# AkshayThiru/distributed-aerial-transportation

Measured on AMD Instinct MI355X. Metric: agent-QP solves/sec (node) + ms per control step, 6-quad C-ADMM, 1/2/4/8 GPU, higher is better.
Workload: dtype f64

## Files before the change

distributed_aerial_transportation_amd/_lib.py:

```python

from __future__ import annotations

import ctypes
import hashlib
import os
import subprocess

import numpy as np

PKG = os.path.dirname(os.path.abspath(__file__))
REPO = os.path.dirname(PKG)
LIB_PATH = os.path.join(PKG, "libdat.so")
SRC = os.path.join(PKG, "csrc", "dat.hip")
SRC_CENT = os.path.join(PKG, "csrc", "dat_cent.hip")
SRC_COMM = os.path.join(PKG, "csrc", "dat_comm.hip")
SRCS = (SRC, SRC_CENT, SRC_COMM)
OBJ_DIR = os.path.join(PKG, "build")
HIPFLAGS = ["--offload-arch=gfx950", "-O3", "-std=c++17", "-fPIC", "-ffp-contract=on"]
DEPS = [SRC, SRC_CENT, SRC_COMM, os.path.join(PKG, "csrc", "dat_core.hpp"), os.path.join(PKG, "csrc", "dat_qp.hpp"),
        os.path.join(PKG, "csrc", "dat_cadmm_step.hpp"), os.path.join(PKG, "csrc", "dat_dd_step.hpp"),
        os.path.join(PKG, "csrc", "dat_pmrl_step.hpp"), os.path.join(PKG, "csrc", "dat_kargs.hpp"),
        os.path.join(PKG, "csrc", "dat_ckpt.hpp"),
        os.path.join(PKG, "csrc", "dat_layout.h"), os.path.join(REPO, "include", "dat.h")]

# ... 103 lines not shown
    "dat_create": (ctypes.c_int, [ctypes.POINTER(Config), ctypes.POINTER(H)]),
    "dat_destroy": (ctypes.c_int, [H]),
    "dat_last_error": (ctypes.c_char_p, []),
    "dat_device_count": (ctypes.c_int, []),
    "dat_set_params": (ctypes.c_int, [H, D, ctypes.c_int]),
    "dat_set_forests": (ctypes.c_int, [H, ctypes.c_int, I, D, I, D]),
    "dat_set_tolerance": (ctypes.c_int, [H, ctypes.c_double, ctypes.c_int]),
    "dat_set_max_iter": (ctypes.c_int, [H, ctypes.c_int]),
    "dat_set_qp_tolerance": (ctypes.c_int, [H, ctypes.c_double]),
    "dat_reset_warm_start": (ctypes.c_int, [H]),
    "dat_set_state": (ctypes.c_int, [H, D, I]),
    "dat_get_state": (ctypes.c_int, [H, D, I]),
    "dat_checkpoint_bytes": (ctypes.c_int, [H, ctypes.c_int, LL]),
    "dat_checkpoint_save": (ctypes.c_int, [H, I, ctypes.c_int, ctypes.c_void_p, ctypes.c_longlong]),
    "dat_checkpoint_load": (ctypes.c_int, [H, ctypes.c_void_p, ctypes.c_longlong, I, I, ctypes.c_int]),
    "dat_get_checkpoint_ms": (ctypes.c_int, [H, D, D]),
    "dat_control_step": (ctypes.c_int, [H, D, D, D, I, I, D, U8, D]),
    "dat_rollout": (ctypes.c_int, [H, ctypes.c_int, D]),
    "dat_closed_loop": (ctypes.c_int, [H, ctypes.c_int]),
    "dat_control_steps": (ctypes.c_int, [H, ctypes.c_int, D, D, I, I]),
    "dat_set_sub_batches": (ctypes.c_int, [H, ctypes.c_int]),
    "dat_set_advance_overlap": (ctypes.c_int, [H, ctypes.c_int]),
    "dat_set_step_pipeline": (ctypes.c_int, [H, ctypes.c_int]),
    "dat_get_stream_count": (ctypes.c_int, [H]),
    "dat_get_advance_counts": (ctypes.c_int, [H, LL, LL]),
    "dat_debug_advance_split": (ctypes.c_int, [H, U8]),
    "dat_debug_get_env_class": (ctypes.c_int, [H, D, D, I, I]),
    "dat_get_step_marks": (ctypes.c_int, [H, D, ctypes.c_int]),
    "dat_get_counters": (ctypes.c_int, [H, LL, LL, LL, LL, D]),
    "dat_get_class_counters": (ctypes.c_int, [H, ctypes.c_int, LL, LL, LL, D]),
    "dat_get_class_occupancy": (ctypes.c_int, [H, ctypes.c_int, LL, LL]),
    "dat_reset_counters": (ctypes.c_int, [H]),
    "dat_synchronize": (ctypes.c_int, [H]),
    "dat_set_persistent_blocks": (ctypes.c_int, [H, ctypes.c_int]),
    "dat_cadmm_slots": (ctypes.c_int, [H, ctypes.c_int, I]),
    "dat_cadmm_row_mode": (ctypes.c_int, [ctypes.c_int, ctypes.c_int, ctypes.c_int]),
    "dat_env_rows": (ctypes.c_int, [H, D, D, I, U8, D]),
    "dat_solve_agent_qp_batch": (ctypes.c_int, [H, ctypes.c_int, I, I, D, D, D, D, D, D, I, I, U8, D]),
    "dat_solve_agent_qp_rows_batch": (ctypes.c_int, [H, ctypes.c_int, I, I, D, D, D, D, D, D, D, I, D, I, I, U8, D,
                                                     U8]),
    "dat_set_low_level": (ctypes.c_int, [H, ctypes.c_int]),
    "dat_get_kernel_ms": (ctypes.c_int, [H, D]),
    "dat_get_inband_exits": (ctypes.c_int, [H, LL, LL]),
    "dat_get_refinement_counters": (ctypes.c_int, [H, LL, LL]),
    "dat_get_robust_redos": (ctypes.c_int, [H, LL]),
    "dat_get_tail_counters": (ctypes.c_int, [H, LL]),
# ... 59 lines not shown
```

distributed_aerial_transportation_amd/control.py:

```python

from __future__ import annotations

import ctypes
from dataclasses import dataclass, field
from typing import Any, List, Optional, Tuple

import numpy as np

from . import _lib as L
from . import layout
from .system import (RQPCollision, RQPParameters, RQPState, _skew, equilibrium_forces, pack_mountain, pack_params,
                     pack_state)

MODES = {"centralized": L.MODE_CENTRALIZED, "consensus-admm": L.MODE_CADMM, "cadmm": L.MODE_CADMM,
         "dual-decomposition": L.MODE_DD, "dd": L.MODE_DD}


@dataclass
class SolverStatistics:

    iter: int
    solve_time: float
    collision: bool
    min_env_dist: float
# ... 271 lines not shown
        if f.ndim == 3:
            f = f[None]
        assert f.ndim == 4 and f.shape[1:] == (self.batch, 3, self.n), f.shape
        fd = L.f64(f.transpose(0, 1, 3, 2).reshape(f.shape[0], self.batch, 3 * self.n))
        L.check(self._lib.dat_pmrl_rollout(self._h, int(steps), L.ptr(fd), int(f.shape[0])))

    def pmrl_forward(self, f: np.ndarray):
        B, n = self.batch, self.n
        f = np.asarray(f, float)
        assert f.shape == (B, 3, n), f.shape
        fd = L.f64(f.transpose(0, 2, 1).reshape(B, 3 * n))
        ddq, dvl, dwl, T = np.empty((B, n, 3)), np.empty((B, 3)), np.empty((B, 3)), np.empty((B, n))
        L.check(self._lib.dat_pmrl_forward(self._h, L.ptr(fd), L.ptr(ddq), L.ptr(dvl), L.ptr(dwl), L.ptr(T)))
        return (ddq.transpose(0, 2, 1).copy(), dvl, dwl), T

    def set_sub_batches(self, count: int) -> None:
        L.check(self._lib.dat_set_sub_batches(self._h, int(count)))

    def set_advance_overlap(self, on: bool) -> None:
        L.check(self._lib.dat_set_advance_overlap(self._h, int(bool(on))))

    def set_step_pipeline(self, on: bool) -> None:
        L.check(self._lib.dat_set_step_pipeline(self._h, int(bool(on))))

    def stream_count(self) -> int:
        m = self._lib.dat_get_stream_count(self._h)
        if m < 0:
            L.check(m)
        return m

    def advance_counts(self) -> Tuple[int, int]:
        e, l = ctypes.c_longlong(), ctypes.c_longlong()
        L.check(self._lib.dat_get_advance_counts(self._h, ctypes.byref(e), ctypes.byref(l)))
        return e.value, l.value

    def debug_advance_split(self, early_mask) -> None:
        if early_mask is None:
            L.check(self._lib.dat_debug_advance_split(self._h, None))
            return
        m = np.ascontiguousarray(np.asarray(early_mask) != 0, dtype=np.uint8)
        if m.shape != (self.batch,):
            raise ValueError("early_mask must have one entry per scenario")
        L.check(self._lib.dat_debug_advance_split(self._h, L.ptr(m, L.U8)))

    def debug_env_class(self):
        B, n = self.batch, self.n
# ... 426 lines not shown
```

distributed_aerial_transportation_amd/csrc/dat.hip:

```cpp
#include <hip/hip_runtime.h>

#include <climits>
#include <cmath>
#include <cstdio>
#include <cstring>
#include <cstdlib>
#include <mutex>
#include <string>
#include <type_traits>
#include <vector>
#include <algorithm>
#include <chrono>

#include "../../include/dat.h"
#include "dat_ckpt.hpp"
#include "dat_kargs.hpp"
#include "dat_dd_step.hpp"
#include "dat_pmrl_step.hpp"

using namespace dat;

#ifdef DAT_CAPTURE_LOOSE
namespace dat {
constexpr int CAP_MAX = 64, CAP_DOUBLES = 320;
// ... 156 lines not shown
#pragma unroll
    for (int k = 0; k < ENV_CE; ++k) mine[k] = e[k];
    __syncthreads();
    if (!dead) {
      for (int j = 0; j < n; ++j) {
        const double* q = grp + (size_t)j * ENV_CS;
        if (q[0] == 0.0) continue;
        if (!env_in_cone(cam, q[1], q[2])) continue;
        const double dd = q[3];
        if (dd < ENV_TOUCH) out.collision = 1;
        env_see(seen, dd, q + 4, lhs, rhs);
      }
    }
    __syncthreads();
  }
  if (!dead && seen.cnt > 0 && fr.speed > 0.0) {
    out.min_env_dist = seen.dmin;
    *mask = env_mask(seen);
  }
  return out;
}

template <int ADV>
__global__ __launch_bounds__(64) __attribute__((amdgpu_waves_per_eu(2))) void k_env_class(KArgs a) {
  __shared__ int nd[64], cl[64];
  __shared__ double md[64];
  __shared__ double ent[64 * ENV_CS];
  const int n = a.n, G = 64 / n, NT = G * n;
  const int lane = threadIdx.x;
  const int ls = lane / n, i = lane - ls * n;
  const int sc = blockIdx.x * G + ls;
  const bool valid = (lane < NT) && (sc < a.B) && adv_gate<ADV, false>(a, sc);
  if constexpr (ADV != ADV_ALL)
    if (!__syncthreads_or(valid)) return;
  int need = 0, col = 0;
  double dist = 1e300;
  const double* prm = valid ? prm_of(a, sc) : a.params;
  const double* trees = nullptr;
  int nt = 0;
  if (valid) forest_of(a, sc, &trees, &nt);
  unsigned emask;
  double lhs[DAT_NENV][3], rhs[DAT_NENV];
  EnvOut e = env_rows_coop(prm, n, valid ? a.state + (size_t)sc * a.S : nullptr, trees, nt, i, ls, valid,
                           prm[DAT_P_AENVD], &emask, lhs, rhs, ent);
  if (valid) {
    need = env_class_of(emask, lhs, rhs);
    col = e.collision;
    dist = e.min_env_dist;
    const size_t NA = (size_t)a.B * n, g = (size_t)sc * n + i;
    a.emask[g] = emask;
#pragma unroll
    for (int j = 0; j < DAT_NENV; ++j) {
      if (!((emask >> j) & 1u)) continue;
      a.erows[(4 * j + 0) * NA + g] = lhs[j][0];
      a.erows[(4 * j + 1) * NA + g] = lhs[j][1];
      a.erows[(4 * j + 2) * NA + g] = lhs[j][2];
      a.erows[(4 * j + 3) * NA + g] = rhs[j];
    }
  }
  nd[lane] = need;
  cl[lane] = col;
  md[lane] = dist;
  __syncthreads();
  int cnum = 0;
  double cmin = 1e300;
// ... 5 lines not shown
      c |= cl[ls * n + k];
      m = fmin(m, md[ls * n + k]);
    }
    const int pit = ADV == ADV_EARLY ? ld_wt(a.iters + sc) : a.iters[sc];
    const int pmx = ADV == ADV_EARLY ? ld_wt(a.ipmx + sc) : a.ipmx[sc];
    const int bin = NPB * iter_bin(pit) + ipm_bin(pmx);
    a.need[sc] = a.route && tail_wedged(pit, a.tail_prev) ? NKEY + cls : cls * NIB + (NIB - 1 - bin);
    a.col[sc] = (unsigned char)c;
    a.mind[sc] = m;
    cnum = c;
    cmin = m;
  }
  for (int off = 32; off > 0; off >>= 1) {
    cnum += __shfl_xor(cnum, off);
    cmin = fmin(cmin, __shfl_xor(cmin, off));
  }
  if (lane == 0) {
    if (cnum) atomicAdd(a.counters + CNT_COLL, (unsigned long long)cnum);
    unsigned long long* pm = a.counters + CNT_COLL + 1;
    const unsigned long long key = dist_key(cmin);
    if (cmin == cmin && key < *(volatile unsigned long long*)pm) atomicMin(pm, key);
  }
}

constexpr int BUCKET_T = 1024;
static_assert(NKEY_ALL <= BUCKET_T, "bucket_sort initialises one key per thread");
template <int ADV>
__device__ __forceinline__ void bucket_sort(int B, const int* need, int* list, int* count, const int* adv,
                                            int serial) {
  const auto take = [&](int q) {
    if constexpr (ADV == ADV_ALL) return true;
    else return (adv[q] == serial && need[q] < NKEY) == (ADV == ADV_EARLY);
  };
  __shared__ int hist[NKEY_ALL], kstart[NKEY_ALL], cursor[NKEY_ALL], tot[NKEY_ALL];
  const int t = threadIdx.x;
  if (t < NKEY_ALL) { hist[t] = 0; cursor[t] = 0; }
  __syncthreads();
  for (int q = t; q < B; q += BUCKET_T)
    if (take(q)) atomicAdd(&hist[min(max(need[q], 0), NKEY_ALL - 1)], 1);
  __syncthreads();
  if (t == 0) {
    int st = 0;
    for (int k = 0; k < NKEY_ALL; ++k) { kstart[k] = st; tot[k] = hist[k]; st += hist[k]; }
  }
  __syncthreads();
  for (int q = t; q < B; q += BUCKET_T) {
    if (!take(q)) continue;
    const int key = min(max(need[q], 0), NKEY_ALL - 1);
    list[kstart[key] + atomicAdd(&cursor[key], 1)] = q;
  }
  if (t == 0) {
    int st = 0;
    for (int cl = 0; cl < NCLS; ++cl) {
      int sz = 0;
      for (int b = 0; b < NIB; ++b) sz += tot[cl * NIB + b];
      count[sc_at(SC_SIZE, cl)] = sz;
      count[sc_at(SC_START, cl)] = st;
      count[sc_at(SC_HEAD, cl)] = 0;
      count[sc_at(SC_HAND_SIZE, cl)] = 0;
      count[sc_at(SC_HAND_HEAD, cl)] = 0;
      st += sz;
    }
    for (int cl = 0; cl < NCLS; ++cl) {
      count[sc_at(SC_TAIL_SIZE, cl)] = tot[NKEY + cl];
      count[sc_at(SC_TAIL_START, cl)] = kstart[NKEY + cl];
      count[sc_at(SC_TAIL_HEAD, cl)] = 0;
    }
  }
}
__global__ __launch_bounds__(BUCKET_T) void k_bucket(int B, const int* need, int* list, int* count) {
  bucket_sort<ADV_ALL>(B, need, list, count, nullptr, 0);
}
template <int ADV>
__global__ __launch_bounds__(BUCKET_T) void k_bucket_adv(int B, const int* need, int* list, int* count,
                                                         const int* adv, int serial) {
  static_assert(ADV == ADV_EARLY || ADV == ADV_REST, "the unfiltered sort is k_bucket");
  bucket_sort<ADV>(B, need, list, count, adv, serial);
}

struct WaveCounters {
  long long qp = 0, ipm = 0, rowit = 0;
  long long inband = 0, loose = 0;
  long long refs = 0, corrs = 0;
  long long slot = 0, pass = 0;
  long long cert = 0, stall = 0, warm = 0;
};
__device__ inline unsigned long long wave_sum(long long v) {
  unsigned long long s = (unsigned long long)v;
  for (int off = 32; off > 0; off >>= 1) s += __shfl_xor(s, off);
  return s;
}
__device__ __forceinline__ void flush_solve_counters(const KArgs& a, unsigned long long* cc, const WaveCounters& wc) {
  const unsigned long long q = wave_sum(wc.qp), ip = wave_sum(wc.ipm), rw = wave_sum(wc.rowit);
  const unsigned long long ib = wave_sum(wc.inband), lo = wave_sum(wc.loose);
  const unsigned long long rf = wave_sum(wc.refs), co = wave_sum(wc.corrs);
  if (threadIdx.x == 0) {
    atomicAdd(cc, q);
    atomicAdd(cc + 1, ip);
    atomicAdd(cc + 2, rw);
    if (ib) atomicAdd(a.counters + CNT_INBAND, ib);
// ... 715 lines not shown
            L.wmx[ls] = 0;
          }
        } else if (i == 0) {
          L.sid[ls] = -1;
        }
      }
    }
    __syncthreads();
  }
  flush_solve_counters(a, a.counters, wc);
}

constexpr int RO_X = 6;
constexpr double REF_X_OFFSET = 1.5;
__device__ inline void mountain_of(const KArgs& a, int sc, double* m) {
  const int f = (a.nforest > 0) ? (a.scen_forest ? a.scen_forest[sc] : 0) : -1;
  if (f < 0 || a.mountain == nullptr) {
    m[DAT_M_CX] = 30.0; m[DAT_M_CY] = 0.0; m[DAT_M_RADIUS] = 25.0; m[DAT_M_SPHERE_R] = 1e300; m[DAT_M_DEPTH] = 0.0;
  } else {
    for (int k = 0; k < DAT_MOUNTAIN_SIZE; ++k) m[k] = a.mountain[(size_t)f * DAT_MOUNTAIN_SIZE + k];
  }
}
template <bool LOG, int ADV>
__global__ __launch_bounds__(64) void k_rollout_agents(KArgs a, int steps, double dt, const double* fdes,
                                                       std::conditional_t<LOG, LogArgs, NoLog> lg) {
  static_assert(!LOG || ADV == ADV_ALL, "the logging rollout is not gated");
  __shared__ double xs[64 * RO_X];
  const int n = a.n, G = 64 / n, NT = G * n;
  const int lane = threadIdx.x, ls = lane / n, i = lane - ls * n;
  const int sc = blockIdx.x * G + ls;
  bool valid = lane < NT && sc < a.B;
  if constexpr (ADV != ADV_ALL) {
    valid = __shfl((int)(valid && adv_gate<ADV, true>(a, sc)), (ls * n) & 63) != 0 && valid;
    asm volatile("" ::: "memory");
    const unsigned long long took = __ballot(valid && i == 0);
    if (!took) return;
    if (lane == 0) atomicAdd(a.advcnt + (ADV == ADV_EARLY ? 0 : 1), (unsigned long long)__builtin_popcountll(took));
  }
  const double* prm = valid ? prm_of(a, sc) : a.params;
  double* g = valid ? a.state + (size_t)sc * a.S : nullptr;
  double R[9], W[3], xl[3], vl[3], Rl[9], wl[3], fd[3];
  int cnt = 0;
  if (valid) {
    for (int k = 0; k < 9; ++k) { R[k] = g[DAT_S_R(n) + 9 * i + k]; Rl[k] = g[DAT_S_RL(n) + k]; }
    for (int c = 0; c < 3; ++c) {
      W[c] = g[DAT_S_W(n) + 3 * i + c];
      xl[c] = g[DAT_S_XL(n) + c];
      vl[c] = g[DAT_S_VL(n) + c];
      wl[c] = g[DAT_S_WL(n) + c];
      fd[c] = ADV == ADV_EARLY ? ld_wt(fdes + (size_t)sc * 3 * n + 3 * i + c) : fdes[(size_t)sc * 3 * n + 3 * i + c];
    }
    cnt = a.counter[sc];
  }
  __shared__ int lslot[LOG ? 64 : 1];
  __shared__ double lref[LOG ? 64 / 3 * 6 : 1];
  [[maybe_unused]] int lnext = 0;
  [[maybe_unused]] double* lrec = nullptr;
  if constexpr (LOG) {
    const long long first = (lg.clock + lg.log_every - 1) / lg.log_every;
// ... 85 lines not shown
    }
    if constexpr (LOG) {
      if (s == lnext) {
        lnext += lg.log_every;
        lrec += (size_t)lg.nslot * DAT_LOG_ST_WORDS(n);
      }
    }
    __syncthreads();
  }
  if (valid) {
    for (int k = 0; k < 9; ++k) g[DAT_S_R(n) + 9 * i + k] = R[k];
    for (int c = 0; c < 3; ++c) g[DAT_S_W(n) + 3 * i + c] = W[c];
    if (i == 0) {
      for (int c = 0; c < 3; ++c) {
        g[DAT_S_XL(n) + c] = xl[c];
        g[DAT_S_VL(n) + c] = vl[c];
        g[DAT_S_WL(n) + c] = wl[c];
      }
      for (int k = 0; k < 9; ++k) g[DAT_S_RL(n) + k] = Rl[k];
      a.counter[sc] = cnt;
      if constexpr (ADV == ADV_EARLY) a.adv[sc] = a.serial;
    }
  }
}

void launch_rollout(const KArgs& a, int B, hipStream_t stream, int steps, double dt, const double* fdes,
                    const LogArgs* lg = nullptr, int adv = ADV_ALL) {
  const int G = 64 / a.n;
  const dim3 grid((B + G - 1) / G);
  constexpr auto k_log = k_rollout_agents<true, ADV_ALL>;
  constexpr auto k_all = k_rollout_agents<false, ADV_ALL>;
  constexpr auto k_early = k_rollout_agents<false, ADV_EARLY>;
  constexpr auto k_rest = k_rollout_agents<false, ADV_REST>;
  if (lg)
    hipLaunchKernelGGL(k_log, grid, dim3(64), 0, stream, a, steps, dt, fdes, *lg);
  else
    hipLaunchKernelGGL(adv == ADV_EARLY ? k_early : adv == ADV_REST ? k_rest : k_all, grid, dim3(64), 0, stream, a,
                       steps, dt, fdes, NoLog{});
}

__global__ void k_low_level(KArgs a, const double* fdes, double* fo, double* Mo) {
  const int t = blockIdx.x * blockDim.x + threadIdx.x;
  const int n = a.n;
  if (t >= a.B * n) return;
  const int sc = t / n, i = t - sc * n;
  const double* prm = prm_of(a, sc);
// ... 110 lines not shown
  double q[3] = {0, 0, 1}, dq[3] = {0, 0, 0}, Rl[9], wl[3], fi[3] = {0, 0, 0};
  if (valid) {
    for (int c = 0; c < 3; ++c) {
      q[c] = g[DAT_S_Q(n) + 3 * i + c];
      dq[c] = g[DAT_S_DQ(n) + 3 * i + c];
      wl[c] = g[DAT_S_WL(n) + c];
      fi[c] = f[(size_t)sc * 3 * n + 3 * i + c];
    }
    for (int k = 0; k < 9; ++k) Rl[k] = g[DAT_S_RL(n) + k];
  }
  double T, ddq[3], dvl[3], dwl[3];
  pmrl_lane_forward(prm, n, i, valid, xs + lane * PM_X, xs + ls * n * PM_X, Rl, wl, q, dq, fi, &T, ddq, dvl, dwl);
  if (valid) {
    for (int c = 0; c < 3; ++c) ddq_o[(size_t)sc * 3 * n + 3 * i + c] = ddq[c];
    T_o[(size_t)sc * n + i] = T;
    if (i == 0)
      for (int c = 0; c < 3; ++c) {
        dvl_o[(size_t)sc * 3 + c] = dvl[c];
        dwl_o[(size_t)sc * 3 + c] = dwl[c];
      }
  }
}

template <int ADV>
__global__ void k_desired(KArgs a, double* acc) {
  const int sc = blockIdx.x * blockDim.x + threadIdx.x;
  if (sc >= a.B || !adv_gate<ADV, false>(a, sc)) return;
  const double* st = a.state + (size_t)sc * a.S;
  double* o = acc + (size_t)sc * 6;
  double m[DAT_MOUNTAIN_SIZE];
  mountain_of(a, sc, m);
  desired_accel_forest(st, a.n, m, REF_X_OFFSET, o);
}

__global__ void k_warm(KArgs a) {
  const int sc = blockIdx.x * blockDim.x + threadIdx.x;
  if (sc >= a.B) return;
  const int n = a.n, N3 = 3 * n;
  const double* prm = prm_of(a, sc);
  const double* feq = prm + DAT_P_FEQ(n);
  if (a.cf) {
    for (int i = 0; i < n; ++i)
      for (int c = 0; c < N3; ++c) {
        a.cf[((size_t)sc * n + i) * N3 + c] = feq[c];
        a.clam[((size_t)sc * n + i) * N3 + c] = 0.0;
      }
    for (int c = 0; c < N3; ++c) a.cfbar[(size_t)sc * N3 + c] = feq[c];
  }
  if (a.dlamF) {
    double s3[3] = {0, 0, 0};
    for (int k = 0; k < n; ++k)
      for (int c = 0; c < 3; ++c) s3[c] += feq[3 * k + c];
    for (int c = 0; c < N3; ++c) { a.dlamF[(size_t)sc * N3 + c] = 0.0; a.dlamM[(size_t)sc * N3 + c] = 0.0; }
    for (int i = 0; i < n; ++i) dd_fallback(prm, n, i, s3, a.dprev + ((size_t)sc * n + i) * 9);
  }
// ... 183 lines not shown
      const T t = *(const T*)(rec + x);
      double v[2] = {0.0, 0.0};
      memcpy(v, &t, sizeof(T));
      if ((unsigned)(x - c.ints_off) < (unsigned)CK_INT_WORDS) {
        for (int j = 0; j < U; ++j) {
          const int i0 = 2 * (x + j - c.ints_off);
          if (c.ints[i0]) c.ints[i0][sc] = __double2loint(v[j]);
          if (c.ints[i0 + 1]) c.ints[i0 + 1][sc] = __double2hiint(v[j]);
        }
      } else if (double* p = ck_word(c, sc, x)) {
        *(T*)p = t;
      }
    }
    if (lane == 0 && c.done) c.done[sc] = 0;
    if (lane == 0 && c.adv) c.adv[sc] = 0;
  }
}

}

constexpr int DAT_MAX_SUB = 4;
#ifndef DAT_STEP_PIPELINE_DEFAULT
#define DAT_STEP_PIPELINE_DEFAULT true
#endif
struct dat_log {
  bool open = false;
  int nslot = 0, log_every = 1, hl_cap = 0;
  long long step_cap = 0;
  int* slot = nullptr;
  double *hl = nullptr, *step = nullptr;
  int* sum_iters = nullptr;
  double* sum_mind = nullptr;
  unsigned char* sum_col = nullptr;
  long long clock = 0, hl_base = 0, step_base = 0;
  std::vector<double> hl_ms;
  long long hl_count(int hl_every) const { return clock / hl_every - hl_base; }
  long long step_count() const { return (clock + log_every - 1) / log_every - step_base; }
};
struct side_stream {
  hipStream_t st = nullptr;
  hipEvent_t ev[3] = {};
};
struct dat_handle {
  dat_log log;
  dat_config cfg;
  int P = 0, S = 0;
// ... 29 lines not shown
  long long hl_steps = 0;
  double hl_ms = 0.0;
  std::vector<double> marks;
  double* acc_seq = nullptr;
  size_t acc_seq_cap = 0;
  double* pmrl_buf = nullptr;
  size_t pmrl_cap = 0;
  int nsub = 1;
  side_stream sub[DAT_MAX_SUB];
  std::vector<hipEvent_t> sub_ev;
  hipEvent_t ev_start = nullptr, ev_end = nullptr;
  side_stream tail;
  double* wrec = nullptr;
  bool adv_on = true;
  int serial = 0;
  int *done = nullptr, *adv = nullptr;
  int* qempty = nullptr;
  int* qempty_dev = nullptr;
  unsigned long long* advcnt = nullptr;
  unsigned char* advmask = nullptr;
  side_stream advance;
  bool pipe_on = DAT_STEP_PIPELINE_DEFAULT;
  side_stream pipe;
  int* pipe_lists = nullptr;
  double agent_qp_ms = 0.0;
  int ll_kind = 0;
  double* ck_stage = nullptr;
  int* ck_list = nullptr;
  size_t ck_stage_cap = 0, ck_list_cap = 0;
  double ck_kernel_ms = 0.0, ck_copy_ms = 0.0;
  std::vector<void*> allocs;
  std::vector<hipStream_t> streams;
  std::vector<hipEvent_t> events;
};

#define DAT_ARRAYS_ALL(X, n) X(counter, 1) X(iters, 1) X(acc, 6) X(qstatus, n) X(mind, 1) X(col, 1)
#define DAT_ARRAYS_CADMM(X, n)                                                              \
  X(need, 1) X(ipmx, 1) X(slist, 1) X(rlist, 1) X(done, 1) X(adv, 1) X(rres, RRES_INTS)     \
  X(erows, 4 * DAT_NENV * (n)) X(emask, n) X(wrec, (n) * WREC_SIZE) X(best, (n) * BEST_REC)
#define DAT_ARRAYS_DD(X, n)                                     \
  X(need, 1) X(ipmx, 1) X(slist, 1) X(dHinv, 36 * (n) * (n))    \
  X(wrec, (n) * WREC_SIZE) X(best, (n) * BEST_REC)
#define DAT_ARRAYS_CENT(X, n) X(best, NMAX_CENT * BEST_REC)
#define DAT_ARR_CK(arr, words, off) DAT_ARR(arr, words)
#define DAT_ARRAYS_OF(mode, n)                \
  do {                                        \
// ... 226 lines not shown
  dat_log& g = h->log;
  for (void* p : {(void*)g.slot, (void*)g.hl, (void*)g.step, (void*)g.sum_iters, (void*)g.sum_mind, (void*)g.sum_col})
    (void)hipFree(p);
  g = dat_log();
}

int log_admit(const dat_handle* h, int hl_steps) {
  const dat_log& g = h->log;
  if (!g.open || hl_steps <= 0) return 0;
  const long long held = g.hl_count(h->cfg.hl_every);
  if (held + hl_steps > g.hl_cap)
    return fail("dat_closed_loop: " + std::to_string(hl_steps) + " HL steps on top of the " + std::to_string(held) +
                " held would pass the log's hl_capacity = " + std::to_string(g.hl_cap) +
                " (read the log and dat_log_clear, or open it larger); nothing was run");
  return 0;
}


struct Sub {
  hipStream_t st;
  KArgs a;
  int off;
  hipEvent_t ek, e1;
};
Sub sub_batch(const dat_handle* h, int s = 0, int S = 1) {
  const SubRange r = sub_range(h->cfg.batch, s, S);
  Sub u;
  u.st = h->sub[s].st;
  u.off = r.off;
  u.a = sub_kargs(h, r, s);
  u.ek = h->ek;
  u.e1 = h->e1;
  return u;
}
void adv_args(const dat_handle* h, KArgs& a) {
  a.done = h->done;
  a.adv = h->adv;
  a.qempty = h->qempty_dev;
  a.advmask = h->advmask;
  a.advcnt = h->advcnt;
}

int step_entry(dat_handle* h) {
  if (!h->have_params) return fail("dat_set_params has not been called");
  HIPCHK(hipSetDevice(h->cfg.device));
  if (tail_wanted(h)) (void)side_get(h, &h->tail, 2);
// ... 9 lines not shown
  static const Kernels ks[] = {{k_desired<ADV_ALL>, k_env_class<ADV_ALL>},
                               {k_desired<ADV_EARLY>, k_env_class<ADV_EARLY>},
                               {k_desired<ADV_REST>, k_env_class<ADV_REST>}};
  static_assert(ADV_ALL == 0 && ADV_EARLY == 1 && ADV_REST == 2, "ks is indexed by the mode");
  const int B = u.a.B, G = 64 / u.a.n;
  if (parts & IN_DESIRED)
    hipLaunchKernelGGL(ks[mode].desired, dim3((B + 63) / 64), dim3(64), 0, u.st, u.a, (double*)u.a.acc);
  if ((parts & IN_ENV) && h->cfg.mode == DAT_MODE_CADMM)
    hipLaunchKernelGGL(ks[mode].env_class, dim3((B + G - 1) / G), dim3(64), 0, u.st, u.a);
}

int step_begin(const dat_handle* h, const Sub& u) {
  if (h->cfg.record_err && u.a.err)
    HIPCHK(hipMemsetAsync(u.a.err, 0xff, sizeof(double) * (size_t)u.a.B * (h->cfg.max_iter + 1), u.st));
  HIPCHK(hipEventRecord(h->e0, u.st));
  return 0;
}

int launch_control(const dat_handle* h, const Sub& u, int mode = ADV_ALL, int stamp = 0) {
  const KArgs& a = u.a;
  if (h->cfg.mode == DAT_MODE_CADMM) {
    if (mode == ADV_ALL)
      hipLaunchKernelGGL(k_bucket, dim3(1), dim3(BUCKET_T), 0, u.st, a.B, (const int*)a.need, a.slist, a.scount);
    else
      hipLaunchKernelGGL(mode == ADV_EARLY ? k_bucket_adv<ADV_EARLY> : k_bucket_adv<ADV_REST>, dim3(1),
                         dim3(BUCKET_T), 0, u.st, a.B, (const int*)a.need, a.slist, a.scount, (const int*)a.adv, stamp);
    HIPCHK(hipEventRecord(u.ek, u.st));
    if (launch_cadmm(h, a, std::min((a.B + a.G - 1) / a.G, h->persistent_blocks), u.st)) return -1;
  } else if (h->cfg.mode == DAT_MODE_DD) {
    if (launch_dd(h, a, u.st, u.ek)) return -1;
  } else {
    HIPCHK(launch_cent(a.n, a.B, u.st, a));
  }
  HIPCHK(hipGetLastError());
  HIPCHK(hipEventRecord(u.e1, u.st));
  return 0;
}

int launch_step(const dat_handle* h, const Sub& u, bool timed = true) {
  if (timed && step_begin(h, u)) return -1;
  launch_inputs(h, u, ADV_ALL, IN_ENV);
  return launch_control(h, u);
}

void launch_step_rollout(const dat_handle* h, const Sub& u, int mode = ADV_ALL) {
  const LogArgs lg = h->log.open ? log_args(h, u.off) : LogArgs();
  launch_rollout(u.a, u.a.B, u.st, h->cfg.hl_every, h->cfg.dt, (const double*)u.a.fdes, h->log.open ? &lg : nullptr,
                 mode);
}

double now_ms() {
  return std::chrono::duration<double, std::milli>(std::chrono::steady_clock::now().time_since_epoch()).count();
}

int account(dat_handle* h, hipEvent_t begin, hipEvent_t end, const hipEvent_t* drain, size_t ndrain, int steps,
            double* span_ms = nullptr) {
  HIPCHK(hipEventSynchronize(end));
  float ms = 0.f;
  HIPCHK(hipEventElapsedTime(&ms, begin, end));
  h->hl_ms += ms;
  if (span_ms) *span_ms = ms;
  for (size_t j = 0; j < ndrain; ++j) {
    float mk = 0.f;
    HIPCHK(hipEventElapsedTime(&mk, drain[2 * j], drain[2 * j + 1]));
    h->cadmm_ms += mk;
  }
  h->hl_steps += steps;
  return 0;
}
int account_step(dat_handle* h, const Sub& u, int ksteps = 1, double* step_ms = nullptr) {
  const hipEvent_t drain[2] = {u.ek, u.e1};
// ... 25 lines not shown
int wait_queue_empty(const dat_handle* h, int serial) {
  const volatile int* const qe = h->qempty;
  for (;;) {
    bool hit = false;
    for (int k = 0; k < 256 && !hit; ++k) hit = !h->advmask && *qe == serial;
    if (hit) break;
    const hipError_t q = hipEventQuery(h->e1);
    if (q == hipSuccess) break;
    if (q != hipErrorNotReady) HIPCHK(q);
  }
  (void)hipGetLastError();
  return 0;
}

int next_serial(dat_handle* h) { return h->serial = h->serial == INT_MAX ? 1 : h->serial + 1; }

bool pipeline_ready(dat_handle* h) {
  if (!h->pipe_on || h->cfg.record_err || !advance_ready(h)) return false;
  if (side_get(h, &h->pipe, 3) != hipSuccess) return false;
  if (!h->pipe_lists && dalloc(h, &h->pipe_lists, (size_t)4 * h->cfg.batch)) {
    (void)hipGetLastError();
    return false;
  }
  return true;
}

int closed_loop_pipelined(dat_handle* h, int hl_steps) {
  const int B = h->cfg.batch;
  side_stream* const X[2] = {&h->advance, &h->pipe};
  while (h->sub_ev.size() < 2 * (size_t)hl_steps) {
    hipEvent_t e = nullptr;
    HIPCHK(own_event(h, &e));
    h->sub_ev.push_back(e);
  }
  Sub base = sub_batch(h);
  adv_args(h, base.a);
  const auto main_drain = [&](int k, int serial) {
    Sub m = base;
    if (k > 0) {
      const int j = (k - 1) & 1;
      m.st = X[j]->st;
      m.a.slist = h->pipe_lists + (size_t)2 * j * B;
      m.a.rlist = m.a.slist + B;
      m.a.scount = h->scount + SCOUNT_INTS * (1 + j);
    }
    m.a.serial = serial;
    m.ek = h->sub_ev[2 * (size_t)k];
    m.e1 = h->sub_ev[2 * (size_t)k + 1];
    return m;
  };
  h->marks.assign(1, now_ms());
  int marked = 0;
  const auto mark = [&](int upto) {
    while (marked < upto && hipEventQuery(h->sub_ev[2 * (size_t)marked + 1]) == hipSuccess) {
      h->marks.push_back(now_ms());
      ++marked;
    }
    (void)hipGetLastError();
  };
  HIPCHK(hipEventRecord(h->e0, h->stream));
  launch_inputs(h, base);
  int serial = next_serial(h);
  if (launch_control(h, main_drain(0, serial))) return -1;
  for (int k = 0; k < hl_steps; ++k) {
    const bool more = k + 1 < hl_steps;
    const hipEvent_t e1 = h->sub_ev[2 * (size_t)k + 1];
    for (const volatile int* const qe = h->qempty;;) {
      bool hit = false;
      for (int q = 0; q < 256 && !hit; ++q) hit = !h->advmask && *qe == serial;
      mark(k);
      if (hit) break;
      const hipError_t q = hipEventQuery(e1);
      if (q == hipSuccess) break;
      if (q != hipErrorNotReady) HIPCHK(q);
    }
    (void)hipGetLastError();
    side_stream& x = *X[k & 1];
    Sub early = base;
    early.st = x.st;
    early.a.serial = serial;
    if (k > 0) HIPCHK(hipStreamWaitEvent(x.st, h->pipe.ev[1], 0));
    if (k > 0 && h->advmask) HIPCHK(hipStreamWaitEvent(x.st, h->pipe.ev[2], 0));
    launch_step_rollout(h, early, ADV_EARLY);
    if (more) launch_inputs(h, early, ADV_EARLY);
    HIPCHK(hipEventRecord(x.ev[0], x.st));
    const int next = more ? next_serial(h) : 0;
    if (more && launch_control(h, main_drain(k + 1, next), ADV_EARLY, serial)) return -1;
    Sub rest = base;
    rest.a.serial = serial;
    if (k > 0) HIPCHK(hipStreamWaitEvent(rest.st, e1, 0));
    HIPCHK(hipStreamWaitEvent(rest.st, x.ev[0], 0));
    launch_step_rollout(h, rest, ADV_REST);
    if (more) {
      launch_inputs(h, rest, ADV_REST);
      rest.a.serial = next;
      rest.a.qempty = h->scount + SCOUNT_INTS * 3;
      rest.ek = h->pipe.ev[1];
      rest.e1 = h->pipe.ev[2];
      if (launch_control(h, rest, ADV_REST, serial)) return -1;
    }
    HIPCHK(hipGetLastError());
    serial = next;
  }
  HIPCHK(hipEventRecord(h->e1, h->stream));
  HIPCHK(hipEventSynchronize(h->e1));
  for (side_stream* s : X) HIPCHK(hipStreamSynchronize(s->st));
  if (h->tail.st) HIPCHK(hipStreamSynchronize(h->tail.st));
  mark(hl_steps);
  float ms = 0.f;
  HIPCHK(hipEventElapsedTime(&ms, h->e0, h->e1));
  h->hl_ms += ms;
  for (int k = 0; k < hl_steps; ++k) {
    HIPCHK(hipEventElapsedTime(&ms, h->sub_ev[2 * (size_t)k], h->sub_ev[2 * (size_t)k + 1]));
    h->cadmm_ms += ms;
  }
  h->hl_steps += hl_steps;
  return 0;
// ... 519 lines not shown
      h->sub_ev.push_back(e);
    }
    HIPCHK(hipEventRecord(h->ev_start, h->stream));
    for (int s = 1; s < S; ++s) HIPCHK(hipStreamWaitEvent(u[s].st, h->ev_start, 0));
  }
  for (int k = 0; k < hl_steps; ++k) {
    for (int s = 0; s < S; ++s) {
      Sub& v = u[s];
      if (S > 1) {
        v.ek = h->sub_ev[2 * ((size_t)k * S + s)];
        v.e1 = h->sub_ev[2 * ((size_t)k * S + s) + 1];
      }
      if (!overlap) {
        launch_inputs(h, v, ADV_ALL, IN_DESIRED);
        if (launch_step(h, v, S == 1)) return -1;
        launch_step_rollout(h, v);
      } else {
        if (step_begin(h, v)) return -1;
        if (k == 0) launch_inputs(h, v);
        v.a.serial = next_serial(h);
        if (launch_control(h, v) || wait_queue_empty(h, h->serial)) return -1;
        Sub early = v;
        early.st = h->advance.st;
        launch_step_rollout(h, early, ADV_EARLY);
        if (k + 1 < hl_steps) launch_inputs(h, early, ADV_EARLY);
        HIPCHK(hipEventRecord(h->advance.ev[0], early.st));
        HIPCHK(hipStreamWaitEvent(v.st, h->advance.ev[0], 0));
        launch_step_rollout(h, v, ADV_REST);
        if (k + 1 < hl_steps) launch_inputs(h, v, ADV_REST);
      }
      HIPCHK(hipGetLastError());
    }
    double step_ms = std::nan("");
    if (S == 1 && account_step(h, u[0], 1, &step_ms)) return -1;
    if (h->log.open) {
      h->log.clock += h->cfg.hl_every;
      h->log.hl_ms.push_back(step_ms);
    }
    if (S == 1) h->marks.push_back(now_ms());
  }
  if (S > 1) {
    for (int s = 1; s < S; ++s) {
      HIPCHK(hipEventRecord(h->sub[s].ev[0], u[s].st));
      HIPCHK(hipStreamWaitEvent(h->stream, h->sub[s].ev[0], 0));
    }
    HIPCHK(hipEventRecord(h->ev_end, h->stream));
    if (account(h, h->ev_start, h->ev_end, h->sub_ev.data(), ndrain, hl_steps)) return -1;
    h->marks.push_back(now_ms());
  }
  HIPCHK(hipStreamSynchronize(h->stream));
  return 0;
}
// ... 69 lines not shown
  HIPCHK(hipSetDevice(h->cfg.device));
  if (count > 1)
    for (side_stream* s : {&h->tail, &h->advance, &h->pipe}) side_release(h, s);
  for (int s = count; s < DAT_MAX_SUB; ++s)
    if (s > 0) side_release(h, &h->sub[s]);
  for (int s = 1; s < count; ++s) HIPCHK(side_get(h, &h->sub[s], 1));
  if (count > 1) {
    HIPCHK(own_event(h, &h->ev_start));
    HIPCHK(own_event(h, &h->ev_end));
  }
  h->nsub = count;
  return 0;
}

int dat_set_advance_overlap(dat_handle* h, int on) {
  if (!h) return fail("null handle");
  h->adv_on = on != 0;
  return 0;
}

int dat_set_step_pipeline(dat_handle* h, int on) {
  if (!h) return fail("null handle");
  h->pipe_on = on != 0;
  return 0;
}

int dat_get_stream_count(dat_handle* h) {
  if (!h) return fail("null handle");
  return (int)h->streams.size();
}

int dat_get_advance_counts(dat_handle* h, long long* early, long long* late) {
  if (!h) return fail("null handle");
  return read_words(h, h->advcnt, {early, late});
}

int dat_debug_advance_split(dat_handle* h, const unsigned char* early_mask) {
  if (!h) return fail("null handle");
  if (h->cfg.mode != DAT_MODE_CADMM) return fail("dat_debug_advance_split: C-ADMM handles only");
  HIPCHK(hipSetDevice(h->cfg.device));
  HIPCHK(hipStreamSynchronize(h->stream));
  if (!early_mask) {
    dfree(h, h->advmask);
    h->advmask = nullptr;
    return 0;
  }
// ... 481 lines not shown
```

include/dat.h:

```cpp
#ifndef DAT_H
#define DAT_H

#ifdef __cplusplus
extern "C" {
#endif

#define DAT_MODE_CENTRALIZED 0
#define DAT_MODE_CADMM 1
#define DAT_MODE_DD 2

#define DAT_LL_PD 0
#define DAT_LL_SM 1

#define DAT_QP_OPTIMAL 0
#define DAT_QP_INACCURATE 1
#define DAT_QP_INFEASIBLE 2
#define DAT_QP_FAILED 3

typedef struct dat_handle dat_handle;

typedef struct dat_config {
  int device;
  int mode;
  int n;
// ... 26 lines not shown

int dat_checkpoint_bytes(dat_handle* h, int count, long long* bytes);
int dat_checkpoint_save(dat_handle* h, const int* scenarios, int count, void* blob, long long bytes);
int dat_checkpoint_load(dat_handle* h, const void* blob, long long bytes, const int* records, const int* scenarios,
                        int count);
int dat_get_checkpoint_ms(dat_handle* h, double* kernel_ms, double* copy_ms);

int dat_control_step(dat_handle* h, const double* state, const double* acc_des, double* f_des, int* iters,
                     int* qp_status, double* min_env_dist, unsigned char* collision, double* err_seq);

int dat_control_steps(dat_handle* h, int steps, const double* acc_seq, double* f_des, int* iters, int* qp_status);

int dat_rollout(dat_handle* h, int steps, const double* f_des);
int dat_set_low_level(dat_handle* h, int kind);
int dat_low_level_control(dat_handle* h, const double* f_des, double* thrust, double* moment);
int dat_rp_rollout(dat_handle* h, int steps, const double* f);
int dat_pmrl_rollout(dat_handle* h, int steps, const double* f, int nf);
int dat_pmrl_forward(dat_handle* h, const double* f, double* ddq, double* dvl, double* dwl, double* T);

int dat_closed_loop(dat_handle* h, int hl_steps);
int dat_set_sub_batches(dat_handle* h, int count);
int dat_set_advance_overlap(dat_handle* h, int on);
int dat_set_step_pipeline(dat_handle* h, int on);
int dat_get_stream_count(dat_handle* h);
int dat_get_advance_counts(dat_handle* h, long long* early, long long* late);
int dat_debug_advance_split(dat_handle* h, const unsigned char* early_mask);
int dat_debug_get_env_class(dat_handle* h, double* lhs, double* rhs, int* nrow, int* env_class);
int dat_get_step_marks(dat_handle* h, double* marks_ms, int max_marks);

int dat_log_begin(dat_handle* h, const int* scenarios, int count, int log_every, int hl_capacity, int summary);
int dat_log_counts(dat_handle* h, long long* hl_records, long long* step_records, long long* clock);
int dat_log_read_hl(dat_handle* h, int first, int count, double* f_des, int* iters, int* qp_status, double* min_env_dist,
                    unsigned char* collision, double* x_ref, double* v_ref, double* solve_ms);
int dat_log_read_steps(dat_handle* h, int first, int count, long long* step_index, double* thrust, double* moment,
                       double* state, double* x_err, double* v_err);
int dat_log_read_summary(dat_handle* h, int first, int count, int* iters, double* min_env_dist,
                         unsigned char* collision);
int dat_log_clear(dat_handle* h);
int dat_log_end(dat_handle* h);

int dat_get_counters(dat_handle* h, long long* qp_solves, long long* ipm_iters, long long* ipm_row_iters,
                     long long* hl_steps, double* hl_kernel_ms);
int dat_get_class_counters(dat_handle* h, int env_class, long long* qp_solves, long long* ipm_iters,
                           long long* ipm_row_iters, double* kernel_ms);
int dat_get_class_occupancy(dat_handle* h, int env_class, long long* slot_ipm_iters, long long* wave_admm_iters);
int dat_reset_counters(dat_handle* h);
// ... 41 lines not shown
```

Baseline: 141.5 million.

## Fuse rollout, desired-accel and env-class into one advance kernel with multi-block scatter sort

Adds a k_advance kernel that runs the agent rollout, the desired-acceleration computation and env classification in one launch for the gated early/rest passes. It also accumulates per-key histograms into device tables. A new multi-block k_bucket_scatter then consumes those counts in place of the single-block bucket sort. The aim is to cut kernel launch count and the serial one-block sort on the C-ADMM step pipeline, at the cost of higher shared-memory and register pressure in the fused kernel and more cross-pass table bookkeeping.

```diff
diff --git a/distributed_aerial_transportation_amd/_lib.py b/distributed_aerial_transportation_amd/_lib.py
--- a/distributed_aerial_transportation_amd/_lib.py
+++ b/distributed_aerial_transportation_amd/_lib.py
@@ -149,6 +149,8 @@
     "dat_set_sub_batches": (ctypes.c_int, [H, ctypes.c_int]),
     "dat_set_advance_overlap": (ctypes.c_int, [H, ctypes.c_int]),
     "dat_set_step_pipeline": (ctypes.c_int, [H, ctypes.c_int]),
+    "dat_set_fused_advance": (ctypes.c_int, [H, ctypes.c_int]),
+    "dat_get_fused_launches": (ctypes.c_int, [H, LL, LL]),
     "dat_get_stream_count": (ctypes.c_int, [H]),
     "dat_get_advance_counts": (ctypes.c_int, [H, LL, LL]),
     "dat_debug_advance_split": (ctypes.c_int, [H, U8]),
diff --git a/distributed_aerial_transportation_amd/control.py b/distributed_aerial_transportation_amd/control.py
--- a/distributed_aerial_transportation_amd/control.py
+++ b/distributed_aerial_transportation_amd/control.py
@@ -317,6 +317,14 @@
 
     def set_step_pipeline(self, on: bool) -> None:
         L.check(self._lib.dat_set_step_pipeline(self._h, int(bool(on))))
+
+    def set_fused_advance(self, on: bool) -> None:
+        L.check(self._lib.dat_set_fused_advance(self._h, int(bool(on))))
+
+    def fused_launches(self) -> Tuple[int, int]:
+        a, s = ctypes.c_longlong(), ctypes.c_longlong()
+        L.check(self._lib.dat_get_fused_launches(self._h, ctypes.byref(a), ctypes.byref(s)))
+        return a.value, s.value
 
     def stream_count(self) -> int:
         m = self._lib.dat_get_stream_count(self._h)
diff --git a/distributed_aerial_transportation_amd/csrc/dat.hip b/distributed_aerial_transportation_amd/csrc/dat.hip
--- a/distributed_aerial_transportation_amd/csrc/dat.hip
+++ b/distributed_aerial_transportation_amd/csrc/dat.hip
@@ -202,17 +202,9 @@
 }
 
 template <int ADV>
-__global__ __launch_bounds__(64) __attribute__((amdgpu_waves_per_eu(2))) void k_env_class(KArgs a) {
-  __shared__ int nd[64], cl[64];
-  __shared__ double md[64];
-  __shared__ double ent[64 * ENV_CS];
-  const int n = a.n, G = 64 / n, NT = G * n;
-  const int lane = threadIdx.x;
-  const int ls = lane / n, i = lane - ls * n;
-  const int sc = blockIdx.x * G + ls;
-  const bool valid = (lane < NT) && (sc < a.B) && adv_gate<ADV, false>(a, sc);
-  if constexpr (ADV != ADV_ALL)
-    if (!__syncthreads_or(valid)) return;
+__device__ __forceinline__ void env_class_lanes(const KArgs& a, int n, int lane, int ls, int i, int sc, bool valid,
+                                                int* nd, int* cl, double* md, double* ent, double lhs[DAT_NENV][3],
+                                                double rhs[DAT_NENV]) {
   int need = 0, col = 0;
   double dist = 1e300;
   const double* prm = valid ? prm_of(a, sc) : a.params;
@@ -220,7 +212,6 @@
   int nt = 0;
   if (valid) forest_of(a, sc, &trees, &nt);
   unsigned emask;
-  double lhs[DAT_NENV][3], rhs[DAT_NENV];
   EnvOut e = env_rows_coop(prm, n, valid ? a.state + (size_t)sc * a.S : nullptr, trees, nt, i, ls, valid,
                            prm[DAT_P_AENVD], &emask, lhs, rhs, ent);
   if (valid) {
@@ -272,22 +263,58 @@
     if (cmin == cmin && key < *(volatile unsigned long long*)pm) atomicMin(pm, key);
   }
 }
+template <int ADV>
+__global__ __launch_bounds__(64) __attribute__((amdgpu_waves_per_eu(2))) void k_env_class(KArgs a) {
+  __shared__ int nd[64], cl[64];
+  __shared__ double md[64];
+  __shared__ double ent[64 * ENV_CS];
+  const int n = a.n, G = 64 / n, NT = G * n;
+  const int lane = threadIdx.x;
+  const int ls = lane / n, i = lane - ls * n;
+  const int sc = blockIdx.x * G + ls;
+  const bool valid = (lane < NT) && (sc < a.B) && adv_gate<ADV, false>(a, sc);
+  if constexpr (ADV != ADV_ALL)
+    if (!__syncthreads_or(valid)) return;
+  double lhs[DAT_NENV][3], rhs[DAT_NENV];
+  env_class_lanes<ADV>(a, n, lane, ls, i, sc, valid, nd, cl, md, ent, lhs, rhs);
+}
 
 constexpr int BUCKET_T = 1024;
 static_assert(NKEY_ALL <= BUCKET_T, "bucket_sort initialises one key per thread");
 template <int ADV>
+__device__ __forceinline__ bool sort_takes(int q, const int* need, const int* adv, int serial) {
+  if constexpr (ADV == ADV_ALL) return true;
+  else return (adv[q] == serial && need[q] < NKEY) == (ADV == ADV_EARLY);
+}
+__device__ __forceinline__ void class_table(int* count, const int* tot, const int* kstart) {
+  int st = 0;
+  for (int cl = 0; cl < NCLS; ++cl) {
+    int sz = 0;
+    for (int b = 0; b < NIB; ++b) sz += tot[cl * NIB + b];
+    count[sc_at(SC_SIZE, cl)] = sz;
+    count[sc_at(SC_START, cl)] = st;
+    count[sc_at(SC_HEAD, cl)] = 0;
+    count[sc_at(SC_HAND_SIZE, cl)] = 0;
+    count[sc_at(SC_HAND_HEAD, cl)] = 0;
+    st += sz;
+  }
+  for (int cl = 0; cl < NCLS; ++cl) {
+    count[sc_at(SC_TAIL_SIZE, cl)] = tot[NKEY + cl];
+    count[sc_at(SC_TAIL_START, cl)] = kstart[NKEY + cl];
+    count[sc_at(SC_TAIL_HEAD, cl)] = 0;
+  }
+}
+__device__ __forceinline__ int sort_key(int need) { return min(max(need, 0), NKEY_ALL - 1); }
+template <int ADV>
 __device__ __forceinline__ void bucket_sort(int B, const int* need, int* list, int* count, const int* adv,
                                             int serial) {
-  const auto take = [&](int q) {
-    if constexpr (ADV == ADV_ALL) return true;
-    else return (adv[q] == serial && need[q] < NKEY) == (ADV == ADV_EARLY);
-  };
+  const auto take = [&](int q) { return sort_takes<ADV>(q, need, adv, serial); };
   __shared__ int hist[NKEY_ALL], kstart[NKEY_ALL], cursor[NKEY_ALL], tot[NKEY_ALL];
   const int t = threadIdx.x;
   if (t < NKEY_ALL) { hist[t] = 0; cursor[t] = 0; }
   __syncthreads();
   for (int q = t; q < B; q += BUCKET_T)
-    if (take(q)) atomicAdd(&hist[min(max(need[q], 0), NKEY_ALL - 1)], 1);
+    if (take(q)) atomicAdd(&hist[sort_key(need[q])], 1);
   __syncthreads();
   if (t == 0) {
     int st = 0;
@@ -296,27 +323,10 @@
   __syncthreads();
   for (int q = t; q < B; q += BUCKET_T) {
     if (!take(q)) continue;
-    const int key = min(max(need[q], 0), NKEY_ALL - 1);
+    const int key = sort_key(need[q]);
     list[kstart[key] + atomicAdd(&cursor[key], 1)] = q;
   }
-  if (t == 0) {
-    int st = 0;
-    for (int cl = 0; cl < NCLS; ++cl) {
-      int sz = 0;
-      for (int b = 0; b < NIB; ++b) sz += tot[cl * NIB + b];
-      count[sc_at(SC_SIZE, cl)] = sz;
-      count[sc_at(SC_START, cl)] = st;
-      count[sc_at(SC_HEAD, cl)] = 0;
-      count[sc_at(SC_HAND_SIZE, cl)] = 0;
-      count[sc_at(SC_HAND_HEAD, cl)] = 0;
-      st += sz;
-    }
-    for (int cl = 0; cl < NCLS; ++cl) {
-      count[sc_at(SC_TAIL_SIZE, cl)] = tot[NKEY + cl];
-      count[sc_at(SC_TAIL_START, cl)] = kstart[NKEY + cl];
-      count[sc_at(SC_TAIL_HEAD, cl)] = 0;
-    }
-  }
+  if (t == 0) class_table(count, tot, kstart);
 }
 __global__ __launch_bounds__(BUCKET_T) void k_bucket(int B, const int* need, int* list, int* count) {
   bucket_sort<ADV_ALL>(B, need, list, count, nullptr, 0);
@@ -326,6 +336,51 @@
                                                          const int* adv, int serial) {
   static_assert(ADV == ADV_EARLY || ADV == ADV_REST, "the unfiltered sort is k_bucket");
   bucket_sort<ADV>(B, need, list, count, adv, serial);
+}
+
+constexpr int SCATTER_T = 256;
+constexpr int KT_COUNT = 0, KT_CURSOR = NKEY_ALL, KT_INTS = 2 * NKEY_ALL;
+static_assert(NKEY_ALL <= 3 * 64, "k_bucket_scatter scans three keys per lane of one wavefront");
+static_assert(NKEY_ALL <= SCATTER_T, "k_bucket_scatter claims one key per thread");
+template <int ADV>
+__global__ __launch_bounds__(SCATTER_T) void k_bucket_scatter(int B, const int* need, int* list, int* count,
+                                                              const int* adv, int serial, int* tab, int* other) {
+  static_assert(ADV == ADV_EARLY || ADV == ADV_REST, "the unfiltered sort is k_bucket");
+  __shared__ int kstart[NKEY_ALL], tot[NKEY_ALL], hist[NKEY_ALL], base[NKEY_ALL];
+  const int t = threadIdx.x;
+  if (t < NKEY_ALL) hist[t] = 0;
+  if (t < 64) {
+    int c[3], s = 0;
+    for (int j = 0; j < 3; ++j) {
+      const int k = 3 * t + j;
+      c[j] = k < NKEY_ALL ? tab[KT_COUNT + k] : 0;
+      s += c[j];
+    }
+    int incl = s;
+    for (int off = 1; off < 64; off <<= 1) {
+      const int v = __shfl_up(incl, off);
+      if (t >= off) incl += v;
+    }
+    int st = incl - s;
+    for (int j = 0; j < 3; ++j) {
+      const int k = 3 * t + j;
+      if (k < NKEY_ALL) { kstart[k] = st; tot[k] = c[j]; }
+      st += c[j];
+    }
+  }
+  __syncthreads();
+  const int q = blockIdx.x * SCATTER_T + t;
+  const bool take = q < B && sort_takes<ADV>(q, need, adv, serial);
+  const int key = take ? sort_key(need[q]) : -1;
+  const int rank = take ? atomicAdd(&hist[key], 1) : 0;
+  __syncthreads();
+  if (t < NKEY_ALL && hist[t]) base[t] = atomicAdd(tab + KT_CURSOR + t, hist[t]);
+  __syncthreads();
+  const int pos = take ? kstart[key] + base[key] + rank : -1;
+  if ((unsigned)pos < (unsigned)B) list[pos] = q;
+  if (blockIdx.x == 0 && t == 0) class_table(count, tot, kstart);
+  if (blockIdx.x == gridDim.x - 1)
+    for (int k = t; k < KT_INTS; k += SCATTER_T) other[k] = 0;
 }
 
 struct WaveCounters {
@@ -1087,10 +1142,10 @@
   }
 }
 template <bool LOG, int ADV>
-__global__ __launch_bounds__(64) void k_rollout_agents(KArgs a, int steps, double dt, const double* fdes,
-                                                       std::conditional_t<LOG, LogArgs, NoLog> lg) {
+__device__ __forceinline__ bool rollout_lanes(const KArgs& a, int steps, double dt, const double* fdes,
+                                              const std::conditional_t<LOG, LogArgs, NoLog>& lg, double* xs,
+                                              bool* took_part) {
   static_assert(!LOG || ADV == ADV_ALL, "the logging rollout is not gated");
-  __shared__ double xs[64 * RO_X];
   const int n = a.n, G = 64 / n, NT = G * n;
   const int lane = threadIdx.x, ls = lane / n, i = lane - ls * n;
   const int sc = blockIdx.x * G + ls;
@@ -1099,7 +1154,7 @@
     valid = __shfl((int)(valid && adv_gate<ADV, true>(a, sc)), (ls * n) & 63) != 0 && valid;
     asm volatile("" ::: "memory");
     const unsigned long long took = __ballot(valid && i == 0);
-    if (!took) return;
+    if (!took) return false;
     if (lane == 0) atomicAdd(a.advcnt + (ADV == ADV_EARLY ? 0 : 1), (unsigned long long)__builtin_popcountll(took));
   }
   const double* prm = valid ? prm_of(a, sc) : a.params;
@@ -1231,6 +1286,15 @@
       if constexpr (ADV == ADV_EARLY) a.adv[sc] = a.serial;
     }
   }
+  *took_part = valid;
+  return true;
+}
+template <bool LOG, int ADV>
+__global__ __launch_bounds__(64) void k_rollout_agents(KArgs a, int steps, double dt, const double* fdes,
+                                                       std::conditional_t<LOG, LogArgs, NoLog> lg) {
+  __shared__ double xs[64 * RO_X];
+  bool took;
+  (void)rollout_lanes<LOG, ADV>(a, steps, dt, fdes, lg, xs, &took);
 }
 
 void launch_rollout(const KArgs& a, int B, hipStream_t stream, int steps, double dt, const double* fdes,
@@ -1387,15 +1451,47 @@
   }
 }
 
-template <int ADV>
-__global__ void k_desired(KArgs a, double* acc) {
-  const int sc = blockIdx.x * blockDim.x + threadIdx.x;
-  if (sc >= a.B || !adv_gate<ADV, false>(a, sc)) return;
+__device__ __forceinline__ void desired_of(const KArgs& a, int sc, double* acc) {
   const double* st = a.state + (size_t)sc * a.S;
   double* o = acc + (size_t)sc * 6;
   double m[DAT_MOUNTAIN_SIZE];
   mountain_of(a, sc, m);
   desired_accel_forest(st, a.n, m, REF_X_OFFSET, o);
+}
+template <int ADV>
+__global__ void k_desired(KArgs a, double* acc) {
+  const int sc = blockIdx.x * blockDim.x + threadIdx.x;
+  if (sc >= a.B || !adv_gate<ADV, false>(a, sc)) return;
+  desired_of(a, sc, acc);
+}
+
+template <int ADV>
+__global__ __launch_bounds__(64) __attribute__((amdgpu_waves_per_eu(2))) void k_advance(KArgs a, int steps, double dt,
+                                                                                        const double* fdes,
+                                                                                        double* acc, int* kc_lo,
+                                                                                        int* kc_hi) {
+  static_assert(ADV == ADV_EARLY || ADV == ADV_REST, "the ungated step runs the three kernels");
+  __shared__ double xs[64 * RO_X];
+  __shared__ int nd[64], cl[64];
+  __shared__ double md[64];
+  __shared__ double ent[64 * ENV_CS];
+  const int n = a.n, G = 64 / n;
+  const int lane = threadIdx.x, ls = lane / n, i = lane - ls * n;
+  const int sc = blockIdx.x * G + ls;
+  bool valid;
+  if (!rollout_lanes<false, ADV>(a, steps, dt, fdes, NoLog{}, xs, &valid)) return;
+  __syncthreads();
+  if (valid && i == 0) desired_of(a, sc, acc);
+  double lhs[DAT_NENV][3], rhs[DAT_NENV];
+  env_class_lanes<ADV>(a, n, lane, ls, i, sc, valid, nd, cl, md, ent, lhs, rhs);
+  if (kc_lo == nullptr) return;
+  __shared__ int hist[NKEY_ALL];
+  for (int k = lane; k < NKEY_ALL; k += 64) hist[k] = 0;
+  __syncthreads();
+  if (valid && i == 0) atomicAdd(&hist[sort_key(a.need[sc])], 1);
+  __syncthreads();
+  for (int k = lane; k < NKEY_ALL; k += 64)
+    if (const int c = hist[k]) atomicAdd((k < NKEY ? kc_lo : kc_hi) + KT_COUNT + k, c);
 }
 
 __global__ void k_warm(KArgs a) {
@@ -1625,6 +1721,12 @@
 constexpr int DAT_MAX_SUB = 4;
 #ifndef DAT_STEP_PIPELINE_DEFAULT
 #define DAT_STEP_PIPELINE_DEFAULT true
+#endif
+#ifndef DAT_FUSED_ADVANCE_DEFAULT
+#define DAT_FUSED_ADVANCE_DEFAULT true
+#endif
+#ifndef DAT_FUSED_SORT
+#define DAT_FUSED_SORT 1
 #endif
 struct dat_log {
   bool open = false;
@@ -1700,6 +1802,9 @@
   side_stream advance;
   bool pipe_on = DAT_STEP_PIPELINE_DEFAULT;
   side_stream pipe;
+  bool fused_on = DAT_FUSED_ADVANCE_DEFAULT;
+  mutable long long n_advance = 0, n_scatter = 0;
+  int* ktabs = nullptr;
   int* pipe_lists = nullptr;
   double agent_qp_ms = 0.0;
   int ll_kind = 0;
@@ -1972,6 +2077,7 @@
   KArgs a;
   int off;
   hipEvent_t ek, e1;
+  int *kc_lo = nullptr, *kc_hi = nullptr, *ktab = nullptr, *kzero = nullptr;
 };
 Sub sub_batch(const dat_handle* h, int s = 0, int S = 1) {
   const SubRange r = sub_range(h->cfg.batch, s, S);
@@ -2027,7 +2133,12 @@
   if (h->cfg.mode == DAT_MODE_CADMM) {
     if (mode == ADV_ALL)
       hipLaunchKernelGGL(k_bucket, dim3(1), dim3(BUCKET_T), 0, u.st, a.B, (const int*)a.need, a.slist, a.scount);
-    else
+    else if (u.ktab) {
+      hipLaunchKernelGGL(mode == ADV_EARLY ? k_bucket_scatter<ADV_EARLY> : k_bucket_scatter<ADV_REST>,
+                         dim3((a.B + SCATTER_T - 1) / SCATTER_T), dim3(SCATTER_T), 0, u.st, a.B, (const int*)a.need,
+                         a.slist, a.scount, (const int*)a.adv, stamp, u.ktab, u.kzero);
+      ++h->n_scatter;
+    } else
       hipLaunchKernelGGL(mode == ADV_EARLY ? k_bucket_adv<ADV_EARLY> : k_bucket_adv<ADV_REST>, dim3(1),
                          dim3(BUCKET_T), 0, u.st, a.B, (const int*)a.need, a.slist, a.scount, (const int*)a.adv, stamp);
     HIPCHK(hipEventRecord(u.ek, u.st));
@@ -2052,6 +2163,22 @@
   const LogArgs lg = h->log.open ? log_args(h, u.off) : LogArgs();
   launch_rollout(u.a, u.a.B, u.st, h->cfg.hl_every, h->cfg.dt, (const double*)u.a.fdes, h->log.open ? &lg : nullptr,
                  mode);
+}
+
+bool fused_ready(const dat_handle* h) { return h->fused_on && h->cfg.mode == DAT_MODE_CADMM && !h->log.open; }
+int launch_advance(const dat_handle* h, const Sub& u, int mode, bool inputs) {
+  if (inputs && mode != ADV_ALL && fused_ready(h)) {
+    const int G = 64 / u.a.n;
+    hipLaunchKernelGGL(mode == ADV_EARLY ? k_advance<ADV_EARLY> : k_advance<ADV_REST>, dim3((u.a.B + G - 1) / G),
+                       dim3(64), 0, u.st, u.a, h->cfg.hl_every, h->cfg.dt, (const double*)u.a.fdes, (double*)u.a.acc,
+                       u.kc_lo, u.kc_hi);
+    ++h->n_advance;
+    return 0;
+  }
+  if (inputs && u.kc_lo) return fail("launch_advance: a key table was handed to a pass that runs the three kernels");
+  launch_step_rollout(h, u, mode);
+  if (inputs) launch_inputs(h, u, mode);
+  return 0;
 }
 
 double now_ms() {
@@ -2123,6 +2250,10 @@
     (void)hipGetLastError();
     return false;
   }
+  if (!h->ktabs && dalloc(h, &h->ktabs, (size_t)4 * KT_INTS)) {
+    (void)hipGetLastError();
+    return false;
+  }
   return true;
 }
 
@@ -2136,6 +2267,10 @@
   }
   Sub base = sub_batch(h);
   adv_args(h, base.a);
+  const bool fsort = fused_ready(h) && DAT_FUSED_SORT;
+  const auto main_tab = [&](int k) { return fsort ? h->ktabs + KT_INTS * (k & 1) : nullptr; };
+  const auto rest_tab = [&](int k) { return fsort ? h->ktabs + KT_INTS * (2 + (k & 1)) : nullptr; };
+  if (fsort) HIPCHK(hipMemsetAsync(h->ktabs, 0, sizeof(int) * 4 * KT_INTS, h->stream));
   const auto main_drain = [&](int k, int serial) {
     Sub m = base;
     if (k > 0) {
@@ -2144,6 +2279,8 @@
       m.a.slist = h->pipe_lists + (size_t)2 * j * B;
       m.a.rlist = m.a.slist + B;
       m.a.scount = h->scount + SCOUNT_INTS * (1 + j);
+      m.ktab = main_tab(k - 1);
+      m.kzero = main_tab(k);
     }
     m.a.serial = serial;
     m.ek = h->sub_ev[2 * (size_t)k];
@@ -2180,20 +2317,22 @@
     Sub early = base;
     early.st = x.st;
     early.a.serial = serial;
+    early.kc_lo = main_tab(k);
+    early.kc_hi = rest_tab(k);
     if (k > 0) HIPCHK(hipStreamWaitEvent(x.st, h->pipe.ev[1], 0));
     if (k > 0 && h->advmask) HIPCHK(hipStreamWaitEvent(x.st, h->pipe.ev[2], 0));
-    launch_step_rollout(h, early, ADV_EARLY);
-    if (more) launch_inputs(h, early, ADV_EARLY);
+    if (launch_advance(h, early, ADV_EARLY, more)) return -1;
     HIPCHK(hipEventRecord(x.ev[0], x.st));
     const int next = more ? next_serial(h) : 0;
     if (more && launch_control(h, main_drain(k + 1, next), ADV_EARLY, serial)) return -1;
     Sub rest = base;
     rest.a.serial = serial;
+    rest.kc_lo = rest.kc_hi = rest.ktab = rest_tab(k);
+    rest.kzero = rest_tab(k + 1);
     if (k > 0) HIPCHK(hipStreamWaitEvent(rest.st, e1, 0));
     HIPCHK(hipStreamWaitEvent(rest.st, x.ev[0], 0));
-    launch_step_rollout(h, rest, ADV_REST);
+    if (launch_advance(h, rest, ADV_REST, more)) return -1;
     if (more) {
-      launch_inputs(h, rest, ADV_REST);
       rest.a.serial = next;
       rest.a.qempty = h->scount + SCOUNT_INTS * 3;
       rest.ek = h->pipe.ev[1];
@@ -2759,12 +2898,10 @@
         if (launch_control(h, v) || wait_queue_empty(h, h->serial)) return -1;
         Sub early = v;
         early.st = h->advance.st;
-        launch_step_rollout(h, early, ADV_EARLY);
-        if (k + 1 < hl_steps) launch_inputs(h, early, ADV_EARLY);
+        if (launch_advance(h, early, ADV_EARLY, k + 1 < hl_steps)) return -1;
         HIPCHK(hipEventRecord(h->advance.ev[0], early.st));
         HIPCHK(hipStreamWaitEvent(v.st, h->advance.ev[0], 0));
-        launch_step_rollout(h, v, ADV_REST);
-        if (k + 1 < hl_steps) launch_inputs(h, v, ADV_REST);
+        if (launch_advance(h, v, ADV_REST, k + 1 < hl_steps)) return -1;
       }
       HIPCHK(hipGetLastError());
     }
@@ -2880,6 +3017,19 @@
 int dat_set_step_pipeline(dat_handle* h, int on) {
   if (!h) return fail("null handle");
   h->pipe_on = on != 0;
+  return 0;
+}
+
+int dat_set_fused_advance(dat_handle* h, int on) {
+  if (!h) return fail("null handle");
+  h->fused_on = on != 0;
+  return 0;
+}
+
+int dat_get_fused_launches(dat_handle* h, long long* advance, long long* scatter) {
+  if (!h) return fail("null handle");
+  if (advance) *advance = h->n_advance;
+  if (scatter) *scatter = h->n_scatter;
   return 0;
 }
 
diff --git a/include/dat.h b/include/dat.h
--- a/include/dat.h
+++ b/include/dat.h
@@ -72,6 +72,8 @@
 int dat_set_sub_batches(dat_handle* h, int count);
 int dat_set_advance_overlap(dat_handle* h, int on);
 int dat_set_step_pipeline(dat_handle* h, int on);
+int dat_set_fused_advance(dat_handle* h, int on);
+int dat_get_fused_launches(dat_handle* h, long long* advance, long long* scatter);
 int dat_get_stream_count(dat_handle* h);
 int dat_get_advance_counts(dat_handle* h, long long* early, long long* late);
 int dat_debug_advance_split(dat_handle* h, const unsigned char* early_mask);
```

New measurement: 146.4 million, median of 6. +3.4%, better.
